# suoych/KEDs

Measured on AMD Instinct MI355X. Metric: query-images/sec (encode+0.5M top-10) ViT-L/14, higher is better.
Workload: dtype bf16/fp16 operands, fp32 accumulate; 1 GPU; ViT-L/14 encode_image (224x224 synthetic, random-init weights) + exact top-10 over a synthetic unit-norm 0.5M x 768 database; batch_per_gpu=128, global_batch=128, db_rows=500000, dim=768, k=10, parallelism=dp1 encoders + 1-way row-sharded scan

## Files before the change

### include/keds_hip.h

```cpp
#ifndef KEDS_HIP_H
#define KEDS_HIP_H

#include <stddef.h>
#include <stdint.h>

#ifdef __cplusplus
extern "C" {
#endif

#define KEDS_OK 0
#define KEDS_E_ARG (-1)
#define KEDS_E_LAUNCH (-2)
#define KEDS_E_WORKSPACE (-3)

#define KEDS_ABI_VERSION 10

int keds_abi_version(void);
const char* keds_build_flags(void);
const char* keds_last_error(void);

int keds_numerics_guard_set(int32_t* device_flag);

#define KEDS_PROF_GEMM 0
#define KEDS_PROF_ATTN 1
// ... 117 lines not shown
int keds_fold_layernorm_mxfp8(const float* W, const float* bias, const float* gamma, const float* beta, int N, int K,
                              int n_pad, void* wq, void* wscale, float* bias_csum, void* stream);

int keds_gemm_set_workspace(void* ptr, size_t bytes);

int keds_gemm_x3(const void* a, int64_t a_plane, int64_t lda, const void* w, int64_t w_plane, const float* bias, void* out,
                 int64_t ldc, int M, int N, int K, int epilogue, int aux_i, int w_exp, void* stream);
int keds_split_f16_pair(const float* x, int64_t ld, int64_t rows, int cols, void* out, int64_t plane, int* overflow, void* stream);
int keds_split_f16_weight(const float* w, int64_t n, int k, void* out, int64_t plane, int* w_exp, void* stream);
int keds_gemm_force_small(int on);
#define KEDS_GEMM_FORM_NONE 0
#define KEDS_GEMM_FORM_SMALL 1
#define KEDS_GEMM_FORM_PAIR 2
#define KEDS_GEMM_FORM_QUAD 3
#define KEDS_GEMM_FORM_QUAD3 4
#define KEDS_GEMM_FLAG_DEFER 1
#define KEDS_GEMM_FLAG_RESID_PROLOGUE 2
int keds_gemm_last_launch(int* info);
int keds_gemm_plan_query(int epilogue, int M, int N, int K, int64_t lda, int64_t ldc, int cus, size_t splitk_bytes, int small_lds,
                         int* info);
int keds_gemm_plan_query_many(int64_t n, const int64_t* cases, int* info);

int keds_layernorm(const float* x, int64_t x_stride, const float* gamma, const float* beta,
                   void* out, int out_f32, int rows, int dim, void* stream);
int keds_layernorm_ex(const float* x, int64_t x_stride, const float* gamma, const float* beta,
                      void* out, int out_type, int rows, int dim, void* stream);

int keds_attention_debug(int variant);
int keds_attention_stamp_buffer(void* buf);

int keds_attention(const void* qkv, void* out, int B, int S, int heads, int causal, void* stream);
int keds_attention_ex(const void* qkv, void* out, int B, int S, int heads, int causal, int q_limit, void* stream);
int keds_attention_mx(const void* qkv, void* out, int B, int S, int heads, int causal, int q_limit, void* q8, void* s8,
                      int q8_rows, void* stream);
int keds_attention_packed(const void* qkv, void* out, int B, int s_max, const int32_t* seq_off, int heads, int causal, void* stream);
int keds_attention_h(const void* qkv, void* out, int B, int S, int heads, int causal, int q_limit, void* stream);
// ... 196 lines not shown
```

### keds_amd/_lib.py

```python
from __future__ import annotations

import ctypes as C
import os
import subprocess
from typing import Optional

import torch

_HERE = os.path.dirname(os.path.abspath(__file__))
LIB_PATH = os.path.join(_HERE, "csrc", "libkeds_hip.so")

ABI_VERSION = 10
METRIC_L2, METRIC_IP = 0, 1
EPI_BIAS_BF16, EPI_BIAS_QGELU_BF16, EPI_BIAS_RELU_BF16, EPI_BIAS_RESID_F32, EPI_BIAS_F32, EPI_PATCH_F32 = range(6)
EPI_LN_BIAS_BF16, EPI_LN_QGELU_BF16, EPI_RESID_STATS_F32, EPI_RESID_STATS_F16 = 6, 7, 8, 9
EPI_LN_BIAS_BF16_H, EPI_LN_QGELU_BF16_H = 10, 11
EPI_BIAS_BF16_HEADF32 = 12
EPI_X3_BIAS_F32, EPI_X3_RESID_F32, EPI_X3_QGELU_PAIR = 13, 14, 15
EPI_LN_BIAS_F16_H, EPI_LN_QGELU_F16_H, EPI_RESID_STATS_F16_H, EPI_BIAS_RESID_F32_H = 16, 17, 18, 19
EPI_BIAS_QGELU_F16_H, EPI_PATCH_F32_H, EPI_BIAS_F32_H = 20, 21, 22
F32_EPI_BIAS, F32_EPI_QGELU, F32_EPI_RESID, F32_EPI_RELU, F32_EPI_PATCH = range(5)
FP8_EPI_BIAS_BF16, FP8_EPI_LN_BIAS_BF16, FP8_EPI_LN_QGELU_MX, FP8_EPI_RESID_STATS_MX, FP8_EPI_RESID_STATS_MX_H = range(5)
PROF_GEMM, PROF_ATTN, PROF_SCAN, PROF_LN, PROF_OTHER = range(5)
SCAN_MAX_K = 128
# ... 125 lines not shown
    "keds_index_search_packed": (i32, [vp, vp, i64, i32, i32, vp, i32, i32, i32, i64, vp, vp, vp, vp, sz, vp]),
    "keds_topk_merge_parts": (i32, [vp, vp, i32, i32, i32, i32, vp, vp, vp]),
    "keds_exchange_pack": (i32, [vp, vp, vp, i32, i32, i32, i32, i64, vp, vp]),
    "keds_exchange_merge": (i32, [vp, i32, i32, i32, i32, i64, i32, vp, vp, vp, vp]),
    "keds_gather_rows": (i32, [vp, i32, vp, i64, vp, vp]),
    "keds_rank_gallery_workspace_bytes": (sz, [i32, i32]),
    "keds_rank_gallery": (i32, [vp, i32, vp, i32, i32, vp, vp, sz, vp]),
    "keds_cirr_target_rank": (i32, [vp, i32, i32, vp, vp, vp, vp, vp, vp]),
    "keds_label_hits": (i32, [vp, i32, i32, vp, vp, C.POINTER(i32), i32, vp, vp, vp]),
    "keds_gemm_bt": (i32, [vp, vp, vp, vp, i32, i32, i32, i32, vp, i32, vp]),
    "keds_gemm_set_workspace": (i32, [vp, sz]),
    "keds_gemm_force_small": (i32, [i32]),
    "keds_gemm_last_launch": (i32, [vp]),
    "keds_gemm_plan_query": (i32, [i32, i32, i32, i32, i64, i64, i32, sz, i32, vp]),
    "keds_gemm_plan_query_many": (i32, [i64, vp, vp]),
    "keds_gemm_x3": (i32, [vp, C.c_int64, C.c_int64, vp, C.c_int64, vp, vp, C.c_int64, i32, i32, i32, i32, i32, i32, vp]),
    "keds_split_f16_pair": (i32, [vp, C.c_int64, C.c_int64, i32, vp, C.c_int64, vp, vp]),
    "keds_split_f16_weight": (i32, [vp, C.c_int64, i32, vp, C.c_int64, C.POINTER(i32), vp]),
    "keds_gemm_bt_ex2": (i32, [vp, i64, vp, vp, vp, i64, i32, i32, i32, i32, vp, i32, vp, vp]),
    "keds_fold_layernorm": (i32, [vp, vp, vp, vp, i32, i32, vp, vp, vp]),
    "keds_rowstats_cast": (i32, [vp, vp, vp, i32, i32, vp]),
    "keds_rowstats_cast_ex": (i32, [vp, vp, i32, vp, i32, i32, vp]),
    "keds_fold_layernorm_ex": (i32, [vp, vp, vp, vp, i32, i32, vp, i32, vp, vp]),
    "keds_mxfp8_scale_bytes": (sz, [i32, i32]),
    "keds_mxfp8_debug": (i32, [i32]),
    "keds_quantize_mxfp8": (i32, [vp, i32, i32, i32, i32, vp, vp, vp]),
    "keds_gemm_mxfp8": (i32, [vp, vp, i32, vp, vp, i32, vp, vp, i32, i32, i32, vp]),
    "keds_gemm_mxfp8_ex": (i32, [vp, vp, i32, vp, vp, i32, vp, vp, i32, i32, i32, i32, vp, vp, vp, vp, i32, vp]),
    "keds_gemm_mxfp8_last_launch": (i32, [vp]),
    "keds_fold_layernorm_mxfp8": (i32, [vp, vp, vp, vp, i32, i32, i32, vp, vp, vp, vp]),
# ... 197 lines not shown
```

### keds_amd/csrc/elementwise.hip

```cpp
#include "keds_common.h"
#include <math.h>

namespace {

constexpr float LN_EPS = 1e-5f;
constexpr int LN_MAXV = 8;

template <int OUT, int NV>
__global__ __launch_bounds__(256) void layernorm_kernel(const float* __restrict__ x, long long x_stride,
                                                        const int* __restrict__ row_map, int row_mul,
                                                        const float* __restrict__ gamma,
                                                        const float* __restrict__ beta, void* __restrict__ out,
                                                        int rows, int dim, long long pair_plane) {
    const int r = blockIdx.x * 4 + (threadIdx.x >> 6);
    const int lane = threadIdx.x & 63;
    if (r >= rows) return;
    const int rm = row_map ? row_map[r] : 0;
    const bool bad_row = row_map && (unsigned)rm >= (unsigned)row_mul;
    const long long src = (long long)r * row_mul + (bad_row ? 0 : rm);
    const float* p = x + src * x_stride;
    constexpr int MAXV = NV > 0 ? NV : LN_MAXV;
    f32x4 v[MAXV], gg[MAXV], bb[MAXV];
#pragma unroll
    for (int j = 0; j < MAXV; ++j) {
// ... 680 lines not shown
    return keds_align_up((size_t)B, 128) * d * 2;
}

int keds_readout_impl(const float* x, int S, const int32_t* row, const float* gamma, const float* beta,
                      const void* proj_t, float* out, int B, int d, int E, int normalize, void* workspace,
                      size_t workspace_bytes, void* stream, bool f16) {
    KEDS_REQUIRE(x && gamma && beta && proj_t && out && workspace && B > 0, "keds_readout: bad argument");
    KEDS_REQUIRE(ln_dim_ok(d), "keds_readout: d %d unsupported", d);
    if (workspace_bytes < keds_readout_workspace_bytes(B, d)) {
        keds_set_error("keds_readout: workspace too small");
        return KEDS_E_WORKSPACE;
    }
    hipStream_t st = (hipStream_t)stream;
    int rc = keds_layernorm_impl(x, d, row, S, gamma, beta, workspace, f16 ? 2 : 0, B, d, st);
    if (rc) return rc;
    rc = keds_gemm_bt(workspace, proj_t, nullptr, out, B, E, d, f16 ? KEDS_EPI_BIAS_F32_H : KEDS_EPI_BIAS_F32, nullptr, 0, stream);
    if (rc) return rc;
    if (normalize) {
        l2norm_kernel<<<(B + 3) / 4, 256, 0, st>>>(out, out, B, E);
        rc = keds_check_launch("l2norm_kernel");
    }
    return rc;
}

extern "C" int keds_readout(const float* x, int S, const int32_t* row, const float* gamma, const float* beta,
                            const void* proj_t, float* out, int B, int d, int E, int normalize, void* workspace,
                            size_t workspace_bytes, void* stream) {
    return keds_readout_impl(x, S, row, gamma, beta, proj_t, out, B, d, E, normalize, workspace, workspace_bytes, stream, false);
}

// ... 163 lines not shown
```

### keds_amd/csrc/gemm.hip

```cpp
#include "keds_common.h"
#include <math.h>
#include <cstdlib>
#include "gemm_shared.h"
#include "gemm_quad_gen.h"

#ifndef KEDS_QUAD_NOEPI
#define KEDS_QUAD_NOEPI 0
#endif
#ifndef KEDS_QUAD_AUX_X
#define KEDS_QUAD_AUX_X 0
#endif
#ifndef KEDS_QUAD_AUX_W
#define KEDS_QUAD_AUX_W 0
#endif
#ifndef KEDS_QUAD_TIDDMA
#define KEDS_QUAD_TIDDMA 0
#endif

namespace {

constexpr int BM = 128, BN = 128, BK = 64;
constexpr int TILE_BYTES = 128 * BK * 2;
constexpr int BUF_BYTES = 2 * TILE_BYTES;

// ... 629 lines not shown
            bf16x8{(bf16_t)v0[0], (bf16_t)v0[1], (bf16_t)v0[2], (bf16_t)v0[3],
                   (bf16_t)v1[0], (bf16_t)v1[1], (bf16_t)v1[2], (bf16_t)v1[3]};
        row_stats_add(reinterpret_cast<keds_stat_t*>(const_cast<float*>(aux)) + 2 * (size_t)m, sum8(v0, v1),
                      sum8(v0 * v0, v1 * v1), per_row);
    } else if constexpr (epi_resid16(EPI)) {
        f16x8* o = reinterpret_cast<f16x8*>(reinterpret_cast<f16_t*>(out) + (size_t)m * ldc + n);
        const f16x8 r = *o;
        v0 += f32x4{(float)r[0], (float)r[1], (float)r[2], (float)r[3]} + b0;
        v1 += f32x4{(float)r[4], (float)r[5], (float)r[6], (float)r[7]} + b1;
        *o = f16x8{(f16_t)v0[0], (f16_t)v0[1], (f16_t)v0[2], (f16_t)v0[3], (f16_t)v1[0], (f16_t)v1[1], (f16_t)v1[2], (f16_t)v1[3]};
        keds_stat_t* stats = reinterpret_cast<keds_stat_t*>(const_cast<float*>(aux));
        if (stats) row_stats_add(stats + 2 * (size_t)m, sum8(v0, v1), sum8(v0 * v0, v1 * v1), per_row);
    } else {
        epilogue_store<epi_base(EPI)>(v0 + b0, v1 + b1, out, m, n, N, aux, aux_i, ldc, guard);
    }
}



namespace pr {
constexpr int TM = 256, TN = 256, TK = 64;
constexpr int OP_BYTES = 256 * 128;
constexpr int PBUF_BYTES = 2 * OP_BYTES;
constexpr int SIDE_OFF = 2 * PBUF_BYTES;
constexpr int LDS_BYTES = SIDE_OFF + 4096;
}

template <int EPI, int STAMP = 0, int RP = 0>
__global__ __launch_bounds__(512, 2) void gemm_bt_pair_kernel(const bf16_t* __restrict__ X, const bf16_t* __restrict__ W,
                                                              const float* __restrict__ bias, void* __restrict__ out,
// ... 768 lines not shown
        s.small_lds = is("KEDS_SMALL_NST", '2');
        s.quad_defer = !is("KEDS_QUAD_DEFER", '0');
        s.quad = num("KEDS_GEMM_QUAD", s.quad);
        s.resid_quad_min_k = num("KEDS_RESID_QUAD_K", s.resid_quad_min_k);
        s.x3_quad = !is("KEDS_X3_QUAD", '0');
        s.big_tiles_pct = num("KEDS_BIG_TILES_PCT", s.big_tiles_pct);
        return s;
    }();
    return env;
}
GemmSwitches& gemm_switches() {
    static GemmSwitches sw = gemm_env_switches();
    return sw;
}
thread_local int tl_small_lds = 0;

struct GemmLaunchRecord {
    int form[2], ring[2], splits[2], persistent, flags;
    void info(int out[8]) const {
        const int v[8] = {form[0], form[1], ring[0], ring[1], splits[0], splits[1], persistent, flags};
        for (int i = 0; i < 8; ++i) out[i] = v[i];
    }
};
thread_local GemmLaunchRecord tl_rec = {};
thread_local int tl_rec_slot = 0;
inline void rec_launch(int form, int ring, int splits, int persistent = 0, int flags = 0) {
    tl_rec.form[tl_rec_slot] = form;
    tl_rec.ring[tl_rec_slot] = ring;
    tl_rec.splits[tl_rec_slot] = splits;
    if (tl_rec_slot == 0) {
// ... 32 lines not shown
    if (int rc = keds_func_lds_once((const void*)gemm_bt_kernel<EPI, NST>, NST * BUF_BYTES, "gemm_bt_kernel")) return rc;
    const int m_tiles = (a.M + BM - 1) / BM, n_tiles = a.N / BN;
    const int tiles = m_tiles * n_tiles, splits = p.splits;
    const int m_pad = m_tiles * BM;
    rec_launch(KEDS_GEMM_FORM_SMALL, NST, splits);
    KEDS_LAUNCH((gemm_bt_kernel<EPI, NST>), tiles * splits, 256, NST * BUF_BYTES, a.st, (const bf16_t*)a.A, (const bf16_t*)a.W, a.bias, a.out,
                a.M, a.N, a.K, n_tiles, a.aux, a.aux_i, a.splitk, a.K / splits, tiles, m_pad, a.lda, a.ldc, a.aux2, (int*)nullptr, 0LL, 0LL);
    if (int rc = keds_check_launch("gemm_bt_kernel(split-K)")) return rc;
    const int threads = a.M * (a.N / 8);
    KEDS_LAUNCH((gemm_splitk_reduce_kernel<EPI>), (threads + 255) / 256, 256, 0, a.st, (const float*)a.splitk, splits, m_pad, a.bias, a.out, a.M,
                a.N, a.K, a.aux, a.aux_i, a.ldc, a.aux2, keds_numerics_guard());
    return keds_check_launch("gemm_splitk_reduce_kernel");
}

template <int EPI>
int launch_pair(const GemmArgs& a, const GemmPlan::Part& p) {
    const int m_tiles = a.M / pr::TM, n_tiles = a.N / pr::TN;
    if constexpr (epi_resid16(EPI)) {
        if (p.flags & KEDS_GEMM_FLAG_RESID_PROLOGUE) {
            if (int rc = keds_func_lds_once((const void*)gemm_bt_pair_kernel<EPI, 0, 1>, pr::LDS_BYTES, "gemm_bt_pair_kernel")) return rc;
            rec_launch(KEDS_GEMM_FORM_PAIR, 2, 1, 0, KEDS_GEMM_FLAG_RESID_PROLOGUE);
            KEDS_LAUNCH((gemm_bt_pair_kernel<EPI, 0, 1>), m_tiles * n_tiles, 512, pr::LDS_BYTES, a.st, (const bf16_t*)a.A, (const bf16_t*)a.W,
                        a.bias, a.out, a.M, a.N, a.K, n_tiles, a.aux, a.aux_i, a.aux2, keds_numerics_guard(), 0LL, 0LL);
            return keds_check_launch("gemm_bt_pair_kernel");
        }
    }
    if (int rc = keds_func_lds_once((const void*)gemm_bt_pair_kernel<EPI>, pr::LDS_BYTES, "gemm_bt_pair_kernel")) return rc;
    rec_launch(KEDS_GEMM_FORM_PAIR, 2, 1);
    KEDS_LAUNCH((gemm_bt_pair_kernel<EPI>), m_tiles * n_tiles, 512, pr::LDS_BYTES, a.st, (const bf16_t*)a.A, (const bf16_t*)a.W, a.bias, a.out,
                a.M, a.N, a.K, n_tiles, a.aux, a.aux_i, a.aux2, keds_numerics_guard(), a.a_plane, a.w_plane);
// ... 25 lines not shown
int launch_quad3(const GemmArgs& a, const GemmPlan::Part&) {
    const int n_tiles = a.N / pr::TN, ntiles = (a.M / pr::TM) * n_tiles;
    if (int rc = keds_func_lds_once((const void*)gemm_bt_quad3_kernel<EPI>, 5 * pr::OP_BYTES, "gemm_bt_quad3_kernel")) return rc;
    rec_launch(KEDS_GEMM_FORM_QUAD3, 3, 1);
    KEDS_LAUNCH((gemm_bt_quad3_kernel<EPI>), ntiles, 256, 5 * pr::OP_BYTES, a.st, (const bf16_t*)a.A, (const bf16_t*)a.W, a.bias, a.out, a.M,
                a.N, a.K, n_tiles, a.aux, ntiles);
    return keds_check_launch("gemm_bt_quad3_kernel");
}

template <int EPI>
int launch_part(const GemmArgs& a, const GemmPlan::Part& p) {
    switch (p.form) {
        case KEDS_GEMM_FORM_SMALL:
            if (p.splits > 1) return p.ring == 4 ? launch_splitk<EPI, 4>(a, p) : launch_splitk<EPI, 2>(a, p);
            return p.ring == 4 ? launch_small<EPI, 4>(a, p) : launch_small<EPI, 2>(a, p);
        case KEDS_GEMM_FORM_PAIR: return launch_pair<EPI>(a, p);
        case KEDS_GEMM_FORM_QUAD: return p.persistent ? launch_quad_persistent<EPI>(a, p) : launch_quad<EPI>(a, p);
        case KEDS_GEMM_FORM_QUAD3:
            if constexpr (epi_resid16(EPI)) return launch_quad3<EPI>(a, p);
            else break;
        default: break;
    }
    keds_set_error("keds_gemm_bt: no kernel of form %d for epilogue %d", p.form, EPI);
    return KEDS_E_LAUNCH;
}

template <int EPI>
bool launch_unplanned(const GemmArgs& a, const GemmSwitches& sw, int* rc) {
#ifdef KEDS_EXPERIMENTS
    if constexpr (EPI == KEDS_EPI_LN_BIAS_BF16_H || EPI == KEDS_EPI_LN_QGELU_BF16_H) {
// ... 48 lines not shown
    return false;
}

template <int EPI>
int launch_gemm(GemmArgs a) {
    const int M = a.M, N = a.N, K = a.K;
    KedsProfScope prof(KEDS_PROF_GEMM, a.st,  true);
    prof.work(2.0 * M * N * K);
    tl_rec = GemmLaunchRecord{};
    tl_rec_slot = 0;
    const GemmSwitches& sw = gemm_switches();
    const GemmPlanNeeds needs = gemm_plan_needs(EPI, M, N, K, a.lda, a.ldc, sw);
    size_t splitk_bytes = 0;
    if (needs.splitk) keds_splitk_scratch(&a.splitk, &splitk_bytes);
    if (!a.splitk) splitk_bytes = 0;
    const GemmPlan plan = gemm_plan(EPI, M, N, K, a.lda, a.ldc, needs.cus ? keds_device_cus() : 0, splitk_bytes, tl_small_lds != 0, sw);

    a.M = plan.main.rows;
    int rc = KEDS_OK;
    const bool planned = plan.main.form == KEDS_GEMM_FORM_SMALL || !launch_unplanned<EPI>(a, sw, &rc);
    if (planned) rc = launch_part<EPI>(a, plan.main);
    if (rc) return rc;
    if (plan.tail.form != KEDS_GEMM_FORM_NONE) {
        tl_rec_slot = 1;
        const size_t m_main = plan.main.rows;
        const size_t esz = (epi_base(EPI) == KEDS_EPI_BIAS_RESID_F32 || epi_base(EPI) == KEDS_EPI_BIAS_F32 || EPI == KEDS_EPI_RESID_STATS_F32)
                               ? 4 : 2;
        if constexpr (epi_is_ln(EPI)) {
            a.aux = (const float*)((const keds_stat_t*)a.aux + 2 * m_main);
            if (a.aux2) a.aux2 = (keds_stat_t*)a.aux2 + 2 * m_main;
        } else if constexpr (EPI == KEDS_EPI_RESID_STATS_F32) {
            a.aux = (const float*)((const keds_stat_t*)a.aux + 2 * m_main);
            a.aux2 = (char*)a.aux2 + m_main * N * 2;
        } else if constexpr (epi_resid16(EPI)) {
            if (a.aux) a.aux = (const float*)((const keds_stat_t*)a.aux + 2 * m_main);
// ... 8 lines not shown
    tl_rec.info(got);
    for (int i = 0; planned && i < 8; ++i) {
        if (got[i] != want[i]) {
            keds_set_error("keds_gemm_bt: launched form differs from the plan at [%d]: %d, planned %d (epilogue %d, %d x %d x %d)", i, got[i],
                           want[i], EPI, M, N, K);
            return KEDS_E_LAUNCH;
        }
    }
    return KEDS_OK;
}

}

bool keds_gemm_splits_rows(int M, int N, int K) { return gemm_big_tiles_fill(M, N, K, gemm_switches()) && M % 256 != 0; }
void keds_gemm_small_lds(int on) { tl_small_lds = on; }

extern "C" int keds_gemm_last_launch(int* info) {
    KEDS_REQUIRE(info, "keds_gemm_last_launch: null pointer");
    tl_rec.info(info);
    return KEDS_OK;
}

extern "C" int keds_gemm_force_small(int on) {
    gemm_switches() = gemm_switches_decode(on, gemm_env_switches());
    return KEDS_OK;
}

static int gemm_check_shape(const char* who, int M, int N, int K, int64_t lda, int64_t ldc, int epilogue) {
    KEDS_REQUIRE(M > 0 && N > 0 && K > 0, "%s: empty problem", who);
    KEDS_REQUIRE(N % BN == 0, "%s: N=%d must be a multiple of %d", who, N, BN);
    KEDS_REQUIRE(K % BK == 0, "%s: K=%d must be a multiple of %d", who, K, BK);
    KEDS_REQUIRE(lda >= K && ldc >= N && lda % 8 == 0 && ldc % 8 == 0, "%s: bad row strides", who);
    KEDS_REQUIRE(epi_base(epilogue) != KEDS_EPI_PATCH_F32 || ldc == N, "%s: EPI_PATCH needs a dense output", who);
    return KEDS_OK;
}

extern "C" int keds_gemm_plan_query(int epilogue, int M, int N, int K, int64_t lda, int64_t ldc, int cus, size_t splitk_bytes,
                                    int small_lds, int* info) {
    KEDS_REQUIRE(info, "keds_gemm_plan_query: null pointer");
    KEDS_REQUIRE(epilogue >= 0 && epilogue <= KEDS_EPI_BIAS_F32_H, "keds_gemm_plan_query: unknown epilogue %d", epilogue);
    if (int rc = gemm_check_shape("keds_gemm_plan_query", M, N, K, lda, ldc, epilogue)) return rc;
    gemm_plan(epilogue, M, N, K, lda, ldc, cus, splitk_bytes, small_lds != 0, gemm_switches()).info(info);
    return KEDS_OK;
}

extern "C" int keds_gemm_plan_query_many(int64_t n, const int64_t* cases, int* info) {
    KEDS_REQUIRE(n >= 0 && (n == 0 || (cases && info)), "keds_gemm_plan_query_many: bad argument");
    for (int64_t i = 0; i < n; ++i) {
        const int64_t* c = cases + 9 * i;
        if (int rc = keds_gemm_plan_query((int)c[0], (int)c[1], (int)c[2], (int)c[3], c[4], c[5], (int)c[6], (size_t)c[7], (int)c[8], info + 8 * i))
            return rc;
    }
    return KEDS_OK;
}

extern "C" int keds_gemm_bt_ex2(const void* A, int64_t lda, const void* W, const float* bias, void* out, int64_t ldc,
                                int M, int N, int K, int epilogue, const float* aux, int aux_i, void* aux2, void* stream) {
    KEDS_REQUIRE(A && W && out, "keds_gemm_bt: null pointer");
// ... 67 lines not shown
```

### keds_amd/csrc/gemm_plan.h

```cpp
#pragma once
#include <stddef.h>
#include "../../include/keds_hip.h"

namespace {

constexpr bool epi_x3(int e) { return e == KEDS_EPI_X3_BIAS_F32 || e == KEDS_EPI_X3_RESID_F32 || e == KEDS_EPI_X3_QGELU_PAIR; }
constexpr bool epi_ln_h(int e) {
    return e == KEDS_EPI_LN_BIAS_BF16_H || e == KEDS_EPI_LN_QGELU_BF16_H || e == KEDS_EPI_LN_BIAS_F16_H || e == KEDS_EPI_LN_QGELU_F16_H;
}
constexpr bool epi_h16(int e) {
    return e == KEDS_EPI_LN_BIAS_F16_H || e == KEDS_EPI_LN_QGELU_F16_H || e == KEDS_EPI_RESID_STATS_F16_H || e == KEDS_EPI_BIAS_RESID_F32_H ||
           e == KEDS_EPI_BIAS_QGELU_F16_H || e == KEDS_EPI_PATCH_F32_H || e == KEDS_EPI_BIAS_F32_H;
}
constexpr bool epi_f16(int e) { return epi_ln_h(e) || epi_x3(e) || epi_h16(e); }
constexpr bool epi_is_ln(int e) { return e == KEDS_EPI_LN_BIAS_BF16 || e == KEDS_EPI_LN_QGELU_BF16 || epi_ln_h(e); }
constexpr bool epi_resid16(int e) { return e == KEDS_EPI_RESID_STATS_F16 || e == KEDS_EPI_RESID_STATS_F16_H; }
constexpr int EPI_INT_BIAS_F16 = 100;
constexpr int epi_base(int e) {
    return (e == KEDS_EPI_LN_BIAS_BF16 || e == KEDS_EPI_LN_BIAS_BF16_H)     ? KEDS_EPI_BIAS_BF16
           : (e == KEDS_EPI_LN_QGELU_BF16 || e == KEDS_EPI_LN_QGELU_BF16_H) ? KEDS_EPI_BIAS_QGELU_BF16
           : e == KEDS_EPI_LN_BIAS_F16_H                                    ? EPI_INT_BIAS_F16
           : e == KEDS_EPI_LN_QGELU_F16_H                                   ? KEDS_EPI_BIAS_QGELU_F16_H
           : e == KEDS_EPI_X3_BIAS_F32 || e == KEDS_EPI_BIAS_F32_H          ? KEDS_EPI_BIAS_F32
           : e == KEDS_EPI_X3_RESID_F32 || e == KEDS_EPI_BIAS_RESID_F32_H   ? KEDS_EPI_BIAS_RESID_F32
// ... 4 lines not shown
constexpr bool epi_out_f16(int e) { return epi_base(e) == EPI_INT_BIAS_F16 || epi_base(e) == KEDS_EPI_BIAS_QGELU_F16_H; }

struct GemmSwitches {
    bool force_small = false;
    bool skip_tail = false;
    bool no_split = false;
    bool resid_prologue = false;
    int quad = -1;
    int stamp = 0;
    bool quad3 = true;
    bool quad_defer = true;
    int resid_quad_min_k = 1024;
    bool x3_quad = true;
    int big_tiles_pct = 85;
    bool small_lds = false;
};

inline GemmSwitches gemm_switches_decode(int bits, const GemmSwitches& base) {
    GemmSwitches s = base;
    s.force_small = bits & 1;
    s.skip_tail = (bits >> 8) & 1;
    s.no_split = base.no_split || ((bits >> 9) & 1);
    s.resid_prologue = (bits >> 10) & 1;
    const int q = (bits >> 11) & 3;
    if (q) s.quad = q == 3 ? 0 : q;
    s.stamp = (bits >> 13) & 7;
    s.quad3 = !((bits >> 16) & 1);
    s.quad_defer = base.quad_defer && !((bits >> 17) & 1);
    return s;
}

struct GemmPlan {
    struct Part {
        int form = KEDS_GEMM_FORM_NONE;
        int ring = 0;
        int splits = 0;
        int rows = 0;
        int persistent = 0;
        int workgroups = 0;
        int defer = 0;
        int flags = 0;
    };
    Part main;
// ... 38 lines not shown
    const long m_tiles = (rows + 127) / 128, tiles = m_tiles * (N / 128);
    small_lds = small_lds || sw.small_lds;
    if (gemm_may_split(epi, rows, N, K, sw)) {
        int splits = 1;
        while (splits < 16 && tiles * splits * 2 <= 256 && K % (splits * 2 * 64) == 0 && K / (splits * 2) >= 128) splits *= 2;
        if (splits > 1 && (size_t)splits * (m_tiles * 128) * N * sizeof(float) <= splitk_bytes) {
            p.splits = splits;
            p.ring = small_lds ? 2 : 4;
            return p;
        }
    }
    p.ring = tiles <= 256 && !small_lds ? 4 : 2;
    return p;
}

struct GemmPlanNeeds {
    bool cus, splitk;
};
inline GemmPlanNeeds gemm_plan_needs(int epi, int M, int N, int K, long long lda, long long ldc, const GemmSwitches& sw) {
    const bool big = gemm_big_tiles(epi, M, N, K, lda, ldc, sw);
    const int small_rows = big ? (sw.skip_tail ? 0 : M % 256) : M;
    return GemmPlanNeeds{big && gemm_quad_mode(epi, K, sw) == 2, small_rows > 0 && gemm_may_split(epi, small_rows, N, K, sw)};
}

inline GemmPlan gemm_plan(int epi, int M, int N, int K, long long lda, long long ldc, int cus, size_t splitk_bytes, bool small_lds,
                          const GemmSwitches& sw) {
    GemmPlan plan;
    if (!gemm_big_tiles(epi, M, N, K, lda, ldc, sw)) {
        plan.main = gemm_plan_small(epi, M, N, K, splitk_bytes, small_lds, sw);
        return plan;
    }
    GemmPlan::Part& p = plan.main;
    p.rows = M / 256 * 256;
    p.ring = 2;
    p.splits = 1;
    const int quad = gemm_quad_mode(epi, K, sw);
    const int tiles = (p.rows / 256) * (N / 256);
    const int T = (cus > 256 ? 256 : cus) & ~7;
    if (quad == 2 && tiles > T && T >= 8 && !epi_resid16(epi) && epi != KEDS_EPI_X3_RESID_F32) {
        p.form = KEDS_GEMM_FORM_QUAD;
        p.persistent = 1;
        p.workgroups = T;
        p.defer = epi_is_ln(epi) && sw.quad_defer;
        if (p.defer && !epi_qgelu(epi) && K / 64 >= 8) p.flags = KEDS_GEMM_FLAG_DEFER;
    } else if (quad && epi_resid16(epi) && sw.quad3 && K >= 1024 && K / 64 >= 4) {
        p.form = KEDS_GEMM_FORM_QUAD3;
        p.ring = 3;
    } else if (quad) {
        p.form = KEDS_GEMM_FORM_QUAD;
    } else {
        p.form = KEDS_GEMM_FORM_PAIR;
        if (epi_resid16(epi) && sw.resid_prologue) p.flags = KEDS_GEMM_FLAG_RESID_PROLOGUE;
    }
    if (p.rows != M && !sw.skip_tail) plan.tail = gemm_plan_small(epi, M - p.rows, N, K, splitk_bytes, small_lds, sw);
    return plan;
}

}
```

### keds_amd/csrc/keds_common.h

```cpp
#pragma once
#include <hip/hip_runtime.h>
#include <hip/hip_ext.h>
#include <stdint.h>
#include <stddef.h>
#include "../../include/keds_hip.h"

typedef __bf16 bf16_t;
typedef __attribute__((ext_vector_type(8))) __bf16 bf16x8;
typedef __attribute__((ext_vector_type(4))) __bf16 bf16x4;
typedef __attribute__((ext_vector_type(2))) __bf16 bf16x2;
typedef _Float16 f16_t;
typedef __attribute__((ext_vector_type(8))) _Float16 f16x8;
typedef __attribute__((ext_vector_type(4))) float f32x4;
typedef __attribute__((ext_vector_type(16))) float f32x16;
typedef __attribute__((ext_vector_type(4))) unsigned int u32x4;
typedef __attribute__((ext_vector_type(2))) unsigned int u32x2;

#define KEDS_WAVE 64

#include <cstdlib>
#ifdef KEDS_EXPERIMENTS
inline const char* keds_exp_env(const char* name) { return getenv(name); }
#else
inline const char* keds_exp_env(const char*) { return nullptr; }
// ... 69 lines not shown

#define KEDS_SPLITK_BYTES ((size_t)8 << 20)
struct KedsSplitKScope {
    float* prev_p;
    size_t prev_bytes;
    bool prev_off;
    KedsSplitKScope(void* p, size_t bytes);
    ~KedsSplitKScope();
};
void keds_splitk_scratch(float** p, size_t* bytes);

int* keds_numerics_guard();

bool keds_gemm_splits_rows(int M, int N, int K);
void keds_gemm_small_lds(int on);

#ifndef KEDS_ST_LN
#define KEDS_ST_LN 3
#endif
#ifndef KEDS_ST_RESID
#define KEDS_ST_RESID 0
#endif
#ifndef KEDS_ST_ATTN
#define KEDS_ST_ATTN 0
#endif
#ifndef KEDS_ST_FP8_BF16
#define KEDS_ST_FP8_BF16 0
#endif
#ifndef KEDS_ST_FP8_MX
#define KEDS_ST_FP8_MX 0
// ... 123 lines not shown
```

### keds_amd/csrc/towers.hip

```cpp
#include "keds_common.h"
#include <cstdlib>

int keds_layernorm_impl(const float* x, long long x_stride, const int* row_map, int row_mul, const float* gamma,
                        const float* beta, void* out, int out_f32, int rows, int dim, hipStream_t st);
int keds_cls_rows_impl(float* x, const float* cls, const float* pos, int B, int S, int d, hipStream_t st);
int keds_cast_rows_f16_f32_impl(const void* x16, float* x32, int rows, int dim, long long stride, hipStream_t st);
int keds_gather_rows_impl(const void* src, void* dst, const int32_t* row, int S, int B, int dim, int mode, hipStream_t st,
                          bool global_rows = false);
int keds_embed_tokens_impl(const int32_t* tokens, const float* table, const float* pos, const float* img_tokens,
                           int n_tok, int insert_col, float* x, int B, int L, int Lx, int d, void* stream,
                           const int32_t* seq_off = nullptr);

size_t keds_tower_f32_workspace_bytes(int width, int seq, int B);
int keds_tower_forward_f32(const keds_tower_params* p, float* x, int B, void* ws, hipStream_t st, const int32_t* last_rows = nullptr,
                           const PackedRows* pk = nullptr, const KedsTaps* tp = nullptr);
size_t keds_readout_f32_workspace_bytes(int B, int d);
int keds_readout_f32(const float* x, int S, const int32_t* row, const float* gamma, const float* beta, const float* proj_t,
                     float* out, int B, int d, int E, int normalize, void* workspace, hipStream_t st);
int keds_readout_impl(const float* x, int S, const int32_t* row, const float* gamma, const float* beta, const void* proj_t,
                      float* out, int B, int d, int E, int normalize, void* workspace, size_t workspace_bytes, void* stream, bool f16);

namespace {

size_t pad_rows(size_t m) { return keds_align_up(m, 256); }
// ... 99 lines not shown
}
int attention16(bool h, const void* qkv, void* out, int B, int S, int heads, int causal, int q_limit, hipStream_t st) {
    return h ? keds_attention_h(qkv, out, B, S, heads, causal, q_limit, st) : keds_attention_ex(qkv, out, B, S, heads, causal, q_limit, st);
}
int attention16_packed(bool h, const void* qkv, void* out, int B, int s_max, const int32_t* off, int heads, int causal, hipStream_t st) {
    return h ? keds_attention_packed_h(qkv, out, B, s_max, off, heads, causal, st)
             : keds_attention_packed(qkv, out, B, s_max, off, heads, causal, st);
}

int cls_rows_tail(const keds_tower_params* p, const keds_block_params& k, const TowerWs& t, float* x, const void* x16, int B,
                  hipStream_t st) {
    const int w = p->width, S = p->seq;
    const long long ld = (long long)S * w;
    const bool h = p->f16;
    const int resid = h ? KEDS_EPI_BIAS_RESID_F32_H : KEDS_EPI_BIAS_RESID_F32;
    int rc;
    if (x16 && (rc = keds_cast_rows_f16_f32_impl(x16, x, B, w, ld, st))) return rc;
    if ((rc = attention16(h, t.qkv, t.att, B, S, p->heads, p->causal, 1, st))) return rc;
    if ((rc = keds_gemm_bt_ex(t.att, ld, k.out_w, k.out_b, x, ld, B, w, w, resid, nullptr, 0, st))) return rc;
    if ((rc = keds_layernorm_impl(x, w, nullptr, S, k.ln2_g, k.ln2_b, t.h, h ? 2 : 0, B, w, st))) return rc;
    if ((rc = keds_gemm_bt(t.h, k.fc_w, k.fc_b, t.hid, B, 4 * w, w, h ? KEDS_EPI_BIAS_QGELU_F16_H : KEDS_EPI_BIAS_QGELU_BF16, nullptr, 0,
                           st)))
        return rc;
    return keds_gemm_bt_ex(t.hid, 4 * w, k.proj_w, k.proj_b, x, ld, B, w, 4 * w, resid, nullptr, 0, st);
}

int rows_tail(const keds_tower_params* p, const keds_block_params& k, const TowerWs& t, float* x, const void* x16, int B,
              const int32_t* rows, hipStream_t st, const PackedRows* pk = nullptr) {
    const int w = p->width, S = p->seq;
    const bool h = p->f16;
    const int resid = h ? KEDS_EPI_BIAS_RESID_F32_H : KEDS_EPI_BIAS_RESID_F32;
    int rc;
    if (pk) rc = attention16_packed(h, t.qkv, t.att, B, S, pk->off, p->heads, p->causal, st);
    else rc = attention16(h, t.qkv, t.att, B, S, p->heads, p->causal, S, st);
    if (rc) return rc;
    bf16_t* att_c = t.qkv;
    float* x_c = (float*)((char*)t.qkv + (size_t)B * w * 2);
    const int bound = pk ? pk->valid : S;
    if ((rc = keds_gather_rows_impl(t.att, att_c, rows, bound, B, w, 0, st, pk != nullptr))) return rc;
    if ((rc = keds_gather_rows_impl(x16 ? x16 : (const void*)x, x_c, rows, bound, B, w, x16 ? 1 : 2, st, pk != nullptr))) return rc;
    if ((rc = keds_gemm_bt_ex(att_c, w, k.out_w, k.out_b, x_c, w, B, w, w, resid, nullptr, 0, st))) return rc;
    if ((rc = keds_layernorm_impl(x_c, w, nullptr, 1, k.ln2_g, k.ln2_b, t.h, h ? 2 : 0, B, w, st))) return rc;
    if ((rc = keds_gemm_bt(t.h, k.fc_w, k.fc_b, t.hid, B, 4 * w, w, h ? KEDS_EPI_BIAS_QGELU_F16_H : KEDS_EPI_BIAS_QGELU_BF16, nullptr, 0,
                           st)))
        return rc;
    if ((rc = keds_gemm_bt_ex(t.hid, 4 * w, k.proj_w, k.proj_b, x_c, w, B, w, 4 * w, resid, nullptr, 0, st))) return rc;
// ... 31 lines not shown
    }
    const int fill = (256 - M % 256) % 256;
    return g_tower_fill && fill && bf16_rows_split(M, w) && (long)fill * 64 <= M ? fill : 0;
}
#else
constexpr int tower_fill_rows(int, int) { return 0; }
#endif

int tower_forward_fp8(const keds_tower_params* p, float* x, int B, const TowerWs& t, int Mm, hipStream_t st,
                      const int32_t* last_rows, const KedsTaps* tp) {
    const int w = p->width, S = p->seq;
    const int M = B * S, Mt = M - Mm;
    RowLanes lanes;
    int rc;
    if ((rc = lanes.init(st, Mt > 0))) return rc;
    const RowSpan rem{(size_t)Mm, Mt, lanes.side};
    if ((rc = keds_rowstats_cast_ex(x, t.h, 1, (float*)t.st1, M, w, st))) return rc;
    if ((rc = keds_quantize_mxfp8(x, 0, Mm, w, Mm, t.xq, t.xs, st))) return rc;
    if ((rc = lanes.to_side())) return rc;
    for (int l = 0; l < p->layers; ++l) {
        const keds_block_params& k = p->blocks[l];
        const bool last = l == p->layers - 1;
        if ((rc = keds_gemm_mxfp8_ex(t.xq, t.xs, Mm, k.qkv_q8, k.qkv_s8, 3 * w, k.qkv_bc8, t.qkv, Mm, 3 * w, w,
                                     KEDS_FP8_EPI_LN_BIAS_BF16, (float*)t.st1, (float*)t.st2, nullptr, nullptr, 0, st)))
            return rc;
        if (Mt && (rc = qkv_rows(t, k, w, rem, false))) return rc;
        if ((rc = lanes.to_main())) return rc;
        if (last && last_rows) return rows_tail(p, k, t, x, t.h, B, last_rows, st);
        if (last && p->last_cls_only) return cls_rows_tail(p, k, t, x, t.h, B, st);
        if ((rc = lanes.attention_then_side([&] { return keds_attention_mx(t.qkv, t.att, B, S, p->heads, p->causal, S, t.aq, t.as, Mm, st); })))
// ... 49 lines not shown
    if (pk && pk->rows > pk->valid &&
        hipMemsetAsync(t.att + (size_t)pk->valid * w, 0, (size_t)(pk->rows - pk->valid) * w * sizeof(bf16_t), st) != hipSuccess) {
        keds_set_error("keds_tower_forward: packed rows: %s", hipGetErrorString(hipGetLastError()));
        return KEDS_E_LAUNCH;
    }
    auto attention = [&](hipStream_t s_) {
        return pk ? attention16_packed(h, t.qkv, t.att, B, S, pk->off, p->heads, p->causal, s_)
                  : attention16(h, t.qkv, t.att, B, S, p->heads, p->causal, S, s_);
    };
    if (fp8) return tower_forward_fp8(p, x, B, t, Mm, st, last_rows, tp);
    if (folded) {
        const int fill = allow_fill ? tower_fill_rows(M, w) : 0;
        const bool two = !fill && bf16_rows_split(M, w);
        RowLanes lanes;
        if ((rc = lanes.init(st, two))) return rc;
        const RowSpan body{0, lanes.split ? Mm : M + fill, st};
        const RowSpan rem{(size_t)Mm, lanes.split ? M - Mm : 0, lanes.side};
        if (fill) {
            if (hipMemcpyAsync(x + (size_t)M * w, x, (size_t)fill * w * sizeof(float), hipMemcpyDeviceToDevice, st) != hipSuccess ||
                hipMemsetAsync(t.att + (size_t)M * w, 0, (size_t)fill * w * sizeof(bf16_t), st) != hipSuccess) {
                keds_set_error("keds_tower_forward: filler rows: %s", hipGetErrorString(hipGetLastError()));
                return KEDS_E_LAUNCH;
            }
        }
        if ((rc = keds_rowstats_cast_ex(x, t.h, 1, (float*)t.st1, M + fill, w, st))) return rc;
        if ((rc = lanes.to_side())) return rc;
        const int b_tail = lanes.split && !pk && tail_attention_on_side() ? Mm / S : B;
        const bool tail_side = b_tail > 0 && b_tail < B;
        struct SmallLds {
            bool on;
// ... 367 lines not shown
```

Before: 6757 query-images/sec.

## Add micro GEMM form for small-row tails and CLS-only tower GEMMs

Adds a new wave-level GEMM kernel using 16x64 tiles, deep register prefetch and an optional split of K across waves, for GEMMs with at most 128 rows such as the CLS-only last layer, row tails and the projection. The planner routes these small-row shapes to the micro form, gated by a thread-local scope guard set in the tower and projection paths. The aim is to raise parallelism and cut LDS and tile overhead on tiny-M GEMMs, at the cost of another kernel variant and some planner complexity.

```diff
diff --git a/include/keds_hip.h b/include/keds_hip.h
--- a/include/keds_hip.h
+++ b/include/keds_hip.h
@@ -155,12 +155,16 @@
 #define KEDS_GEMM_FORM_PAIR 2
 #define KEDS_GEMM_FORM_QUAD 3
 #define KEDS_GEMM_FORM_QUAD3 4
+#define KEDS_GEMM_FORM_MICRO 5
 #define KEDS_GEMM_FLAG_DEFER 1
 #define KEDS_GEMM_FLAG_RESID_PROLOGUE 2
 int keds_gemm_last_launch(int* info);
 int keds_gemm_plan_query(int epilogue, int M, int N, int K, int64_t lda, int64_t ldc, int cus, size_t splitk_bytes, int small_lds,
                          int* info);
 int keds_gemm_plan_query_many(int64_t n, const int64_t* cases, int* info);
+int keds_gemm_micro(int level);
+int keds_gemm_plan_query_ex(int epilogue, int M, int N, int K, int64_t lda, int64_t ldc, int cus, size_t splitk_bytes, int small_lds,
+                            int micro, int* info);
 
 int keds_layernorm(const float* x, int64_t x_stride, const float* gamma, const float* beta,
                    void* out, int out_f32, int rows, int dim, void* stream);
diff --git a/keds_amd/_lib.py b/keds_amd/_lib.py
--- a/keds_amd/_lib.py
+++ b/keds_amd/_lib.py
@@ -163,6 +163,8 @@
     "keds_gemm_last_launch": (i32, [vp]),
     "keds_gemm_plan_query": (i32, [i32, i32, i32, i32, i64, i64, i32, sz, i32, vp]),
     "keds_gemm_plan_query_many": (i32, [i64, vp, vp]),
+    "keds_gemm_micro": (i32, [i32]),
+    "keds_gemm_plan_query_ex": (i32, [i32, i32, i32, i32, i64, i64, i32, sz, i32, i32, vp]),
     "keds_gemm_x3": (i32, [vp, C.c_int64, C.c_int64, vp, C.c_int64, vp, vp, C.c_int64, i32, i32, i32, i32, i32, i32, vp]),
     "keds_split_f16_pair": (i32, [vp, C.c_int64, C.c_int64, i32, vp, C.c_int64, vp, vp]),
     "keds_split_f16_weight": (i32, [vp, C.c_int64, i32, vp, C.c_int64, C.POINTER(i32), vp]),
diff --git a/keds_amd/csrc/elementwise.hip b/keds_amd/csrc/elementwise.hip
--- a/keds_amd/csrc/elementwise.hip
+++ b/keds_amd/csrc/elementwise.hip
@@ -718,6 +718,7 @@
     hipStream_t st = (hipStream_t)stream;
     int rc = keds_layernorm_impl(x, d, row, S, gamma, beta, workspace, f16 ? 2 : 0, B, d, st);
     if (rc) return rc;
+    KedsMicroRows micro;
     rc = keds_gemm_bt(workspace, proj_t, nullptr, out, B, E, d, f16 ? KEDS_EPI_BIAS_F32_H : KEDS_EPI_BIAS_F32, nullptr, 0, stream);
     if (rc) return rc;
     if (normalize) {
diff --git a/keds_amd/csrc/gemm.hip b/keds_amd/csrc/gemm.hip
--- a/keds_amd/csrc/gemm.hip
+++ b/keds_amd/csrc/gemm.hip
@@ -667,6 +667,82 @@
     } else {
         epilogue_store<epi_base(EPI)>(v0 + b0, v1 + b1, out, m, n, N, aux, aux_i, ldc, guard);
     }
+}
+
+template <int EPI, int KW>
+__global__ __launch_bounds__(256) void gemm_bt_micro_kernel(const bf16_t* __restrict__ X, const bf16_t* __restrict__ W,
+                                                            const float* __restrict__ bias, void* __restrict__ out, int M, int N, int K,
+                                                            int m_tiles, int units, const float* __restrict__ aux, int aux_i,
+                                                            long long lda, long long ldc, void* __restrict__ aux2,
+                                                            int* __restrict__ guard) {
+    constexpr int D = MICRO_DEPTH;
+    const int lane = threadIdx.x & 63;
+    const int wave = __builtin_amdgcn_readfirstlane(threadIdx.x >> 6);
+    const int g = lane >> 4, c = lane & 15;
+    const int lb = xcd_remap(blockIdx.x, gridDim.x);
+    const int unit = KW > 1 ? lb : lb * (int)(blockDim.x >> 6) + wave;
+    if (KW == 1 && unit >= units) return;
+    const int tn = unit / m_tiles, tm = unit - tn * m_tiles;
+    const int m0 = 16 * tm, n0 = 64 * tn;
+    const int klen = K / KW, k0 = KW > 1 ? wave * klen : 0;
+    const int xr = m0 + c < M ? m0 + c : M - 1;
+    const bf16x8* xp = reinterpret_cast<const bf16x8*>(X + (size_t)xr * lda + k0 + 8 * g);
+    const bf16x8* wp[4];
+#pragma unroll
+    for (int ni = 0; ni < 4; ++ni)
+        wp[ni] = reinterpret_cast<const bf16x8*>(W + (size_t)(n0 + perm_w(16 * ni + c)) * K + k0 + 8 * g);
+
+    f32x4 acc[4][1];
+#pragma unroll
+    for (int ni = 0; ni < 4; ++ni) acc[ni][0] = f32x4{0.f, 0.f, 0.f, 0.f};
+    bf16x8 fx[D], fw[D][4];
+#define KEDS_MICRO_LOAD(j, s)                                                       \
+    {                                                                               \
+        fx[j] = xp[4 * (s)];                                                        \
+        _Pragma("unroll") for (int ni = 0; ni < 4; ++ni) fw[j][ni] = wp[ni][4 * (s)]; \
+    }
+#define KEDS_MICRO_MFMA(j) \
+    _Pragma("unroll") for (int ni = 0; ni < 4; ++ni) acc[ni][0] = mma<epi_f16(EPI)>(fw[j][ni], fx[j], acc[ni][0]);
+    const int nks = klen / 32;
+#pragma unroll
+    for (int j = 0; j < D; ++j)
+        if (j < nks) KEDS_MICRO_LOAD(j, j)
+    int s = 0;
+    for (; s + 2 * D <= nks; s += D) {
+#pragma unroll
+        for (int j = 0; j < D; ++j) {
+            KEDS_MICRO_MFMA(j)
+            KEDS_MICRO_LOAD(j, s + j + D)
+            __builtin_amdgcn_sched_barrier(0);
+        }
+    }
+    for (; s < nks; s += D) {
+#pragma unroll
+        for (int j = 0; j < D; ++j) {
+            if (s + j < nks) {
+                KEDS_MICRO_MFMA(j)
+                if (s + j + D < nks) KEDS_MICRO_LOAD(j, s + j + D)
+            }
+            __builtin_amdgcn_sched_barrier(0);
+        }
+    }
+#undef KEDS_MICRO_LOAD
+#undef KEDS_MICRO_MFMA
+    if constexpr (KW > 1) {
+        __shared__ f32x4 red[KW - 1][4][64];
+        if (wave > 0) {
+#pragma unroll
+            for (int ni = 0; ni < 4; ++ni) red[wave - 1][ni][lane] = acc[ni][0];
+        }
+        __syncthreads();
+        if (wave > 0) return;
+#pragma unroll
+        for (int w = 0; w < KW - 1; ++w)
+#pragma unroll
+            for (int ni = 0; ni < 4; ++ni) acc[ni][0] += red[w][ni][lane];
+    }
+    const bool zl = epi_is_ln(EPI) ? (n0 == 0 && g == 0) : (g == 0);
+    tile_epilogue<EPI, 1>(acc, bias, out, m0 + c, M, n0 + 8 * g, N, K, aux, aux_i, aux2, ldc, zl, guard);
 }
 
 
@@ -1465,6 +1541,7 @@
     return sw;
 }
 thread_local int tl_small_lds = 0;
+thread_local int tl_micro = 0;
 
 struct GemmLaunchRecord {
     int form[2], ring[2], splits[2], persistent, flags;
@@ -1527,6 +1604,22 @@
 }
 
 template <int EPI>
+int launch_micro(const GemmArgs& a, const GemmPlan::Part& p) {
+    const int m_tiles = (a.M + 15) / 16, units = m_tiles * (a.N / 64);
+    if (p.splits > 1) {
+        rec_launch(KEDS_GEMM_FORM_MICRO, MICRO_DEPTH / 2, MICRO_KWAVES);
+        KEDS_LAUNCH((gemm_bt_micro_kernel<EPI, MICRO_KWAVES>), units, 64 * MICRO_KWAVES, 0, a.st, (const bf16_t*)a.A, (const bf16_t*)a.W, a.bias,
+                    a.out, a.M, a.N, a.K, m_tiles, units, a.aux, a.aux_i, a.lda, a.ldc, a.aux2, keds_numerics_guard());
+        return keds_check_launch("gemm_bt_micro_kernel(K over waves)");
+    }
+    const int waves = units <= 256 ? 1 : units <= 512 ? 2 : 4;
+    rec_launch(KEDS_GEMM_FORM_MICRO, MICRO_DEPTH / 2, 1);
+    KEDS_LAUNCH((gemm_bt_micro_kernel<EPI, 1>), (units + waves - 1) / waves, 64 * waves, 0, a.st, (const bf16_t*)a.A, (const bf16_t*)a.W, a.bias,
+                a.out, a.M, a.N, a.K, m_tiles, units, a.aux, a.aux_i, a.lda, a.ldc, a.aux2, keds_numerics_guard());
+    return keds_check_launch("gemm_bt_micro_kernel");
+}
+
+template <int EPI>
 int launch_pair(const GemmArgs& a, const GemmPlan::Part& p) {
     const int m_tiles = a.M / pr::TM, n_tiles = a.N / pr::TN;
     if constexpr (epi_resid16(EPI)) {
@@ -1582,6 +1675,9 @@
         case KEDS_GEMM_FORM_SMALL:
             if (p.splits > 1) return p.ring == 4 ? launch_splitk<EPI, 4>(a, p) : launch_splitk<EPI, 2>(a, p);
             return p.ring == 4 ? launch_small<EPI, 4>(a, p) : launch_small<EPI, 2>(a, p);
+        case KEDS_GEMM_FORM_MICRO:
+            if constexpr (epi_micro(EPI)) return launch_micro<EPI>(a, p);
+            else break;
         case KEDS_GEMM_FORM_PAIR: return launch_pair<EPI>(a, p);
         case KEDS_GEMM_FORM_QUAD: return p.persistent ? launch_quad_persistent<EPI>(a, p) : launch_quad<EPI>(a, p);
         case KEDS_GEMM_FORM_QUAD3:
@@ -1660,11 +1756,11 @@
     size_t splitk_bytes = 0;
     if (needs.splitk) keds_splitk_scratch(&a.splitk, &splitk_bytes);
     if (!a.splitk) splitk_bytes = 0;
-    const GemmPlan plan = gemm_plan(EPI, M, N, K, a.lda, a.ldc, needs.cus ? keds_device_cus() : 0, splitk_bytes, tl_small_lds != 0, sw);
+    const GemmPlan plan = gemm_plan(EPI, M, N, K, a.lda, a.ldc, needs.cus ? keds_device_cus() : 0, splitk_bytes, tl_small_lds != 0, sw, tl_micro);
 
     a.M = plan.main.rows;
     int rc = KEDS_OK;
-    const bool planned = plan.main.form == KEDS_GEMM_FORM_SMALL || !launch_unplanned<EPI>(a, sw, &rc);
+    const bool planned = plan.main.form == KEDS_GEMM_FORM_SMALL || plan.main.form == KEDS_GEMM_FORM_MICRO || !launch_unplanned<EPI>(a, sw, &rc);
     if (planned) rc = launch_part<EPI>(a, plan.main);
     if (rc) return rc;
     if (plan.tail.form != KEDS_GEMM_FORM_NONE) {
@@ -1703,6 +1799,12 @@
 
 bool keds_gemm_splits_rows(int M, int N, int K) { return gemm_big_tiles_fill(M, N, K, gemm_switches()) && M % 256 != 0; }
 void keds_gemm_small_lds(int on) { tl_small_lds = on; }
+extern "C" int keds_gemm_micro(int on) {
+    const int was = tl_micro;
+    tl_micro = on < 0 ? 0 : on > 2 ? 2 : on;
+    return was;
+}
+bool keds_gemm_micro_on_lane() { return gemm_switches().micro_on_lane; }
 
 extern "C" int keds_gemm_last_launch(int* info) {
     KEDS_REQUIRE(info, "keds_gemm_last_launch: null pointer");
@@ -1724,13 +1826,18 @@
     return KEDS_OK;
 }
 
-extern "C" int keds_gemm_plan_query(int epilogue, int M, int N, int K, int64_t lda, int64_t ldc, int cus, size_t splitk_bytes,
-                                    int small_lds, int* info) {
+extern "C" int keds_gemm_plan_query_ex(int epilogue, int M, int N, int K, int64_t lda, int64_t ldc, int cus, size_t splitk_bytes,
+                                       int small_lds, int micro, int* info) {
     KEDS_REQUIRE(info, "keds_gemm_plan_query: null pointer");
     KEDS_REQUIRE(epilogue >= 0 && epilogue <= KEDS_EPI_BIAS_F32_H, "keds_gemm_plan_query: unknown epilogue %d", epilogue);
     if (int rc = gemm_check_shape("keds_gemm_plan_query", M, N, K, lda, ldc, epilogue)) return rc;
-    gemm_plan(epilogue, M, N, K, lda, ldc, cus, splitk_bytes, small_lds != 0, gemm_switches()).info(info);
+    gemm_plan(epilogue, M, N, K, lda, ldc, cus, splitk_bytes, small_lds != 0, gemm_switches(), micro).info(info);
     return KEDS_OK;
+}
+
+extern "C" int keds_gemm_plan_query(int epilogue, int M, int N, int K, int64_t lda, int64_t ldc, int cus, size_t splitk_bytes,
+                                    int small_lds, int* info) {
+    return keds_gemm_plan_query_ex(epilogue, M, N, K, lda, ldc, cus, splitk_bytes, small_lds, 0, info);
 }
 
 extern "C" int keds_gemm_plan_query_many(int64_t n, const int64_t* cases, int* info) {
diff --git a/keds_amd/csrc/gemm_plan.h b/keds_amd/csrc/gemm_plan.h
--- a/keds_amd/csrc/gemm_plan.h
+++ b/keds_amd/csrc/gemm_plan.h
@@ -42,6 +42,9 @@
     bool x3_quad = true;
     int big_tiles_pct = 85;
     bool small_lds = false;
+    bool no_micro = false;
+    bool micro_on_lane = false;
+    bool micro_long_k = false;
 };
 
 inline GemmSwitches gemm_switches_decode(int bits, const GemmSwitches& base) {
@@ -55,6 +58,9 @@
     s.stamp = (bits >> 13) & 7;
     s.quad3 = !((bits >> 16) & 1);
     s.quad_defer = base.quad_defer && !((bits >> 17) & 1);
+    s.no_micro = (bits >> 18) & 1;
+    s.micro_on_lane = (bits >> 19) & 1;
+    s.micro_long_k = (bits >> 20) & 1;
     return s;
 }
 
@@ -123,6 +129,30 @@
     return p;
 }
 
+constexpr int MICRO_MAX_ROWS = 128;
+constexpr int MICRO_DEPTH = 12;
+constexpr int MICRO_KWAVES = 4;
+constexpr bool epi_micro(int e) {
+    return epi_is_ln(e) || epi_resid16(e) || e == KEDS_EPI_BIAS_RESID_F32 || e == KEDS_EPI_BIAS_RESID_F32_H || e == KEDS_EPI_BIAS_QGELU_BF16 ||
+           e == KEDS_EPI_BIAS_QGELU_F16_H || e == KEDS_EPI_BIAS_F32 || e == KEDS_EPI_BIAS_F32_H;
+}
+constexpr long gemm_micro_units(int rows, int N) { return (long)((rows + 15) / 16) * (N / 64); }
+inline bool gemm_micro_ok(int epi, int rows, int N, int K, int micro, const GemmSwitches& sw) {
+    return micro > 0 && !sw.no_micro && epi_micro(epi) && rows <= MICRO_MAX_ROWS && gemm_micro_units(rows, N) <= 1024 &&
+           (K < 2048 || micro >= 2 || sw.micro_long_k);
+}
+inline GemmPlan::Part gemm_plan_micro(int rows, int N, int K, const GemmSwitches& sw) {
+    GemmPlan::Part p;
+    p.form = KEDS_GEMM_FORM_MICRO;
+    p.rows = rows;
+    p.ring = MICRO_DEPTH / 2;
+    p.splits = K >= 2048 && K % (MICRO_KWAVES * 64) == 0 && gemm_micro_units(rows, N) <= 256 && !sw.no_split ? MICRO_KWAVES : 1;
+    return p;
+}
+inline GemmPlan::Part gemm_plan_rows(int epi, int rows, int N, int K, size_t splitk_bytes, bool small_lds, int micro, const GemmSwitches& sw) {
+    return gemm_micro_ok(epi, rows, N, K, micro, sw) ? gemm_plan_micro(rows, N, K, sw) : gemm_plan_small(epi, rows, N, K, splitk_bytes, small_lds, sw);
+}
+
 struct GemmPlanNeeds {
     bool cus, splitk;
 };
@@ -133,10 +163,10 @@
 }
 
 inline GemmPlan gemm_plan(int epi, int M, int N, int K, long long lda, long long ldc, int cus, size_t splitk_bytes, bool small_lds,
-                          const GemmSwitches& sw) {
+                          const GemmSwitches& sw, int micro = 0) {
     GemmPlan plan;
     if (!gemm_big_tiles(epi, M, N, K, lda, ldc, sw)) {
-        plan.main = gemm_plan_small(epi, M, N, K, splitk_bytes, small_lds, sw);
+        plan.main = gemm_plan_rows(epi, M, N, K, splitk_bytes, small_lds, micro, sw);
         return plan;
     }
     GemmPlan::Part& p = plan.main;
@@ -161,7 +191,7 @@
         p.form = KEDS_GEMM_FORM_PAIR;
         if (epi_resid16(epi) && sw.resid_prologue) p.flags = KEDS_GEMM_FLAG_RESID_PROLOGUE;
     }
-    if (p.rows != M && !sw.skip_tail) plan.tail = gemm_plan_small(epi, M - p.rows, N, K, splitk_bytes, small_lds, sw);
+    if (p.rows != M && !sw.skip_tail) plan.tail = gemm_plan_rows(epi, M - p.rows, N, K, splitk_bytes, small_lds, micro, sw);
     return plan;
 }
 
diff --git a/keds_amd/csrc/keds_common.h b/keds_amd/csrc/keds_common.h
--- a/keds_amd/csrc/keds_common.h
+++ b/keds_amd/csrc/keds_common.h
@@ -107,6 +107,14 @@
 
 bool keds_gemm_splits_rows(int M, int N, int K);
 void keds_gemm_small_lds(int on);
+bool keds_gemm_micro_on_lane();
+struct KedsMicroRows {
+    int was;
+    explicit KedsMicroRows(bool on = true) : was(keds_gemm_micro(on ? 1 : 0)) {}
+    ~KedsMicroRows() { keds_gemm_micro(was); }
+    KedsMicroRows(const KedsMicroRows&) = delete;
+    KedsMicroRows& operator=(const KedsMicroRows&) = delete;
+};
 
 #ifndef KEDS_ST_LN
 #define KEDS_ST_LN 3
diff --git a/keds_amd/csrc/towers.hip b/keds_amd/csrc/towers.hip
--- a/keds_amd/csrc/towers.hip
+++ b/keds_amd/csrc/towers.hip
@@ -137,6 +137,7 @@
     const long long ld = (long long)S * w;
     const bool h = p->f16;
     const int resid = h ? KEDS_EPI_BIAS_RESID_F32_H : KEDS_EPI_BIAS_RESID_F32;
+    KedsMicroRows micro;
     int rc;
     if (x16 && (rc = keds_cast_rows_f16_f32_impl(x16, x, B, w, ld, st))) return rc;
     if ((rc = attention16(h, t.qkv, t.att, B, S, p->heads, p->causal, 1, st))) return rc;
@@ -153,6 +154,7 @@
     const int w = p->width, S = p->seq;
     const bool h = p->f16;
     const int resid = h ? KEDS_EPI_BIAS_RESID_F32_H : KEDS_EPI_BIAS_RESID_F32;
+    KedsMicroRows micro;
     int rc;
     if (pk) rc = attention16_packed(h, t.qkv, t.att, B, S, pk->off, p->heads, p->causal, st);
     else rc = attention16(h, t.qkv, t.att, B, S, p->heads, p->causal, S, st);
@@ -214,6 +216,7 @@
     RowLanes lanes;
     int rc;
     if ((rc = lanes.init(st, Mt > 0))) return rc;
+    KedsMicroRows micro(!lanes.split || keds_gemm_micro_on_lane());
     const RowSpan rem{(size_t)Mm, Mt, lanes.side};
     if ((rc = keds_rowstats_cast_ex(x, t.h, 1, (float*)t.st1, M, w, st))) return rc;
     if ((rc = keds_quantize_mxfp8(x, 0, Mm, w, Mm, t.xq, t.xs, st))) return rc;
@@ -293,6 +296,7 @@
         const bool two = !fill && bf16_rows_split(M, w);
         RowLanes lanes;
         if ((rc = lanes.init(st, two))) return rc;
+        KedsMicroRows micro(!lanes.split || keds_gemm_micro_on_lane());
         const RowSpan body{0, lanes.split ? Mm : M + fill, st};
         const RowSpan rem{(size_t)Mm, lanes.split ? M - Mm : 0, lanes.side};
         if (fill) {
```

Result: no change. 6761 query-images/sec (median of 2 runs) (+0.1%).
